# sloisel/MultiGridBarrierMPI.jl

Hardware: AMD Instinct MI355X
Metric: fem2d p-Laplace DoF/s per Newton step (higher is better)
Workload: dtype f64; 1 GPU; fem2d p-Laplace L=7 p=1 (n=57344 rows, N_L=49154 Newton unknowns), amgb main phase, tol=sqrt(eps); parallelism=single GPU

## Files before the change

### multigridbarriermpi.jl_amd/csrc/bwd_fused.cpp

```cpp
#include "bwd_fused.hpp"

#include <algorithm>

#include "chol_plan.hpp"
#include "errors.hpp"

namespace mgb {

namespace {
int round64(int v) { return (v + 63) & ~63; }
}

FusedPlan plan_bwd_fused(const CholTree& T, const FusedKnobs& kn) {
  FusedPlan P;
  const int n = T.size(), nheights = T.nheights;
  const std::vector<int>&ns = T.ns, &nf = T.nf, &first = T.first, &parent = T.parent, &height = T.height, &bofs = T.bofs;
  const std::vector<long long>&off = T.off, &loff = T.loff;
  if (kn.threads < 64 || kn.threads > 512 || (kn.threads & (kn.threads - 1))) throw ArgError("gpuchol: fused backward sweep: bad thread count");
  P.threads = kn.threads;
  P.slots.assign(T.bdry_total, -1);
  if (n == 0) return P;
  std::vector<int> hmax(nheights, 0);
  for (int t = 0; t < n; ++t) hmax[height[t]] = std::max(hmax[height[t]], nf[t]);
  int h_top = -1;
// ... 14 lines not shown
    if (parent[t] >= 0) minfirst[parent[t]] = std::min(minfirst[parent[t]], minfirst[t]);
  for (int t = n - 1; t >= 0; --t) {
    if (height[t] > h_cut) continue;
    if (parent[t] >= 0 && height[parent[t]] <= h_cut) root_of[t] = root_of[parent[t]];
    else root_of[t] = t;
  }
  for (int t = 0; t < n; ++t)
    if (root_of[t] == t) roots.push_back(t);
  std::vector<int> above(n, 0), base(n, 0);
  for (int t = n - 1; t >= 0; --t)
    if (parent[t] >= 0) above[t] = above[parent[t]] + ns[parent[t]];
  for (int t = 0; t < n; ++t) {
    const int r = root_of[t];
    if (r < 0) {
      base[t] = above[t];
      continue;
    }
    if (first[r] + ns[r] - minfirst[r] < 0 || first[t] < minfirst[r] || first[t] + ns[t] > first[r] + ns[r])
      throw InternalError("gpuchol: subtree unknowns are not contiguous");
    base[t] = above[r] + first[t] - minfirst[r];
  }
  for (int t = 0; t < n; ++t) {
    if (height[t] > h_top) continue;
    const std::vector<int>& bd = *T.bdry[t];
    int a = parent[t];
    for (size_t i = 0; i < bd.size(); ++i) {
      while (a >= 0 && !(bd[i] >= first[a] && bd[i] < first[a] + ns[a])) a = parent[a];
      if (a < 0) {
        a = parent[t];
        while (a >= 0 && !(bd[i] >= first[a] && bd[i] < first[a] + ns[a])) a = parent[a];
        if (a < 0) throw InternalError("gpuchol: boundary entry outside the ancestors");
      }
      const int ab = (root_of[a] >= 0) ? base[a] : above[a];
      P.slots[bofs[t] + i] = ab + bd[i] - first[a];
    }
  }
  auto nsl_rect = [&](int t) {
    const int h = height[t], nb = nf[t] - ns[t];
    if (nb == 0 || ns[t] == 0) return 0;
    if (hmax[h] > kn.split_nf) return 1024 / 64;
    const int nt = hmax[h] > 384 ? 1024 : 256;
    return nt / std::min(nt, round64(ns[t]));
  };
  const int W = kn.threads / 64;
  struct Rec {
    std::vector<std::vector<int>> levels;
    int first_solve = 0, sub_level = 0;
  };
  std::vector<Rec> recs(roots.size());
  std::vector<char> stored(n, 0);
  std::vector<std::vector<int>> kids(n);
  for (int t = 0; t < n; ++t)
    if (parent[t] >= 0) kids[parent[t]].push_back(t);
  size_t max_jobs = 0;
  for (size_t w = 0; w < roots.size(); ++w) {
    Rec& R = recs[w];
    const int r = roots[w];
    std::vector<int> anc;
    for (int a = parent[r]; a >= 0; a = parent[a]) anc.push_back(a);
    std::reverse(anc.begin(), anc.end());
    std::vector<int> ab;
    for (int a : anc)
      if (height[a] > h_top) ab.push_back(a);
    if (!ab.empty()) {
      R.levels.push_back(ab);
      R.first_solve = 1;
    }
    for (int a : anc)
      if (height[a] <= h_top) R.levels.push_back({a});
    R.sub_level = (int)R.levels.size();
    std::vector<int> cur{r};
    while (!cur.empty()) {
      R.levels.push_back(cur);
      std::vector<int> nxt;
      for (int t : cur) nxt.insert(nxt.end(), kids[t].begin(), kids[t].end());
      cur.swap(nxt);
    }
    size_t nj = 0;
    for (const auto& l : R.levels) nj += l.size();
    max_jobs = std::max(max_jobs, nj);
    P.max_levels = std::max(P.max_levels, (int)R.levels.size());
  }
  P.h_top = h_top;
  P.h_cut = h_cut;
  P.nwg = (int)roots.size();
  const int jo = kFusedHdr + kFusedLevelInts * P.max_levels;
  P.wstride = jo + kFusedJobInts * (int)max_jobs;
  P.wg.assign((size_t)P.nwg * P.wstride, 0);
  for (size_t w = 0; w < roots.size(); ++w) {
    const Rec& R = recs[w];
    int* rec = P.wg.data() + w * P.wstride;
    const int r = roots[w];
    int nj = 0, sl = 0;
    for (size_t l = 0; l < R.levels.size(); ++l) {
      const std::vector<int>& lv = R.levels[l];
      int* li = rec + kFusedHdr + kFusedLevelInts * l;
      const bool solve = (int)l >= R.first_solve;
      int maxp = 0, items = 0;
      li[0] = nj;
      li[1] = (int)lv.size();
      for (int t : lv) {
        int* j = rec + jo + kFusedJobInts * nj++;
        const int nsl = solve ? nsl_rect(t) : 0;
        int flags = 0;
        if (!solve) flags = 2;
        else if (root_of[t] >= 0 || !stored[t]) {
          flags = 1;
          stored[t] = 1;
        }
        j[FJ_OFF] = (int)(off[t] & 0xffffffffLL);
        j[FJ_OFF + 1] = (int)(off[t] >> 32);
        j[FJ_LOFF] = (int)(loff[t] & 0xffffffffLL);
        j[FJ_LOFF + 1] = (int)(loff[t] >> 32);
        j[FJ_FIRST] = first[t];
        j[FJ_NF] = nf[t];
        j[FJ_NS] = ns[t];
        j[FJ_SOFS] = bofs[t];
        j[FJ_BASE] = base[t];
        j[FJ_LSOFS] = sl;
        j[FJ_NSL] = nsl;
        j[FJ_NT] = hmax[height[t]] > 384 ? 1024 : 256;
        j[FJ_FLAGS] = flags;
        j[FJ_NODE] = t;
        if (solve) {
          sl += nf[t] - ns[t];
          maxp = std::max(maxp, (ns[t] + PB - 1) / PB);
          items = std::max(items, nsl * ns[t]);
        }
      }
      li[2] = maxp;
      li[3] = items;
      if (solve) {
        int G = W;
        while (G > 1 && W / G < (int)lv.size()) G >>= 1;
        P.red_cap = std::max(P.red_cap, (W / G) * items);
      }
    }
    rec[0] = (int)R.levels.size();
    rec[1] = nj;
    rec[2] = R.first_solve;
    rec[3] = above[r] + first[r] + ns[r] - minfirst[r];
    rec[4] = sl;
    rec[5] = R.sub_level;
    P.xs_cap = std::max(P.xs_cap, rec[3]);
    P.sl_cap = std::max(P.sl_cap, sl);
  }
  P.lds_bytes = (size_t)P.wstride * 4 + (size_t)(P.xs_cap + P.red_cap) * 8 + (size_t)P.sl_cap * 4;
  return P;
}

}
```

### multigridbarriermpi.jl_amd/csrc/bwd_fused.hpp

```cpp
#pragma once
#include <cstddef>
#include <vector>

namespace mgb {

struct CholTree;

struct FusedKnobs {
  int cut = 2;
  int max_wg = 256;
  int max_raise = 2;
  int top_nf = 384;
  int threads = 512;
  int split_nf = 192;
};

constexpr int kFusedHdr = 8;
constexpr int kFusedLevelInts = 4;
constexpr int kFusedJobInts = 16;
enum FusedJobField {
  FJ_OFF = 0,
  FJ_LOFF = 2,
  FJ_FIRST = 4,
  FJ_NF = 5,
  FJ_NS = 6,
  FJ_SOFS = 7,
  FJ_BASE = 8,
  FJ_LSOFS = 9,
  FJ_NSL = 10,
  FJ_NT = 11,
  FJ_FLAGS = 12,
  FJ_NODE = 13
};

struct FusedPlan {
  int h_top = -1, h_cut = -1, nwg = 0;
  int wstride = 0;
  int max_levels = 0;
  int xs_cap = 0, sl_cap = 0, red_cap = 0;
  int threads = 0;
  size_t lds_bytes = 0;
  std::vector<int> wg;
  std::vector<int> slots;
  bool enabled() const { return nwg > 0; }
};

FusedPlan plan_bwd_fused(const CholTree& T, const FusedKnobs& kn);

}
```

### multigridbarriermpi.jl_amd/csrc/chol_plan.hpp

```cpp
#pragma once
#include <algorithm>
#include <cstddef>
#include <vector>

#include "bwd_fused.hpp"
#include "chol_premap.hpp"
#include "mfchol.hpp"

namespace mgb {

constexpr int PB = 32;
constexpr int LP = PB + 1;
constexpr int TS = 64;
constexpr int TB = 256;
constexpr int RT = 1024;
constexpr int kStep2Lds = (2 * PB * PB + 3 * PB * LP + 2 * 2 * PB * (TS + 8)) * (int)sizeof(double);
constexpr int kPanel2Lds = (2 * PB * PB + 3 * PB * LP + 2 * PB * (TS + 8)) * (int)sizeof(double);
constexpr int kUpdate2Lds = (2 * 2 * PB * (TS + 8)) * (int)sizeof(double);

struct CholTree {
  int n = 0;
  double flops = 0;
  const std::vector<int>* perm = nullptr;
  std::vector<int> ns, nf, first, parent;
// ... 28 lines not shown
  long long eoff;
};

struct StartJob {
  long long off, loff;
  long long boff[2];
  int cld[2];
  int nf, ns, iofs, first;
  int node, chunk, rb;
  int a0, a1;
  long long soff[2];
};

struct StepTile {
  long long off;
  long long loff;
  int nf, ns;
  short ti, tj;
  int pad;
};

struct SingleTile {
  long long off, loff;
  long long boff[2];
  int cld[2];
  int nf, ns, iofs, a0, a1, first;
  short ti, tj;
  int pld, fofs;
  long long eoff;
  long long soff[2];
};

struct RectJob {
  int node, chunk;
};

struct CholKnobs {
  bool graph = true;
  bool prof = false;
  bool leaf = true;
  bool single = true;
  bool step2 = true;
  bool wide = true;
  bool start_pivot = true;
  int step2_tiles = 224;
  int dense_tiles = 512;
  int bwd_split_nf = 192;
  bool bwd_fused = true;
  int bwd_cut = 2;
  int bwd_fused_nf = 384;
  int bwd_fused_threads = 512;
  int premap = 1;
  int premap_tiles = 400;
};
FusedKnobs fused_knobs(const CholKnobs& kn);

enum class Kind : unsigned char {
  Leaf, Single, SingleNarrow, SingleDense, SingleDenseNarrow, Start, Step, Step2, Panel2, Update2, BwdRect, Bwd256, Bwd1024, BwdFused
};

struct Launch {
  Kind kind;
  int ofs, cnt;
  int block;
  size_t lds;
  int p, npiv;
  bool rect;
  double bytes;
  bool premap = false;
  int nproducers = 0;
};

template <class F>
int for_trailing_tiles(int nf, int k, F&& f) {
  const int Tr = (nf + 1 - k + TS - 1) / TS, Tc = std::max(1, (nf - k + TS - 1) / TS);
  int cnt = 0;
  for (int ti = 0; ti < Tr; ++ti)
    for (int tj = 0; tj <= std::min(ti, Tc - 1); ++tj, ++cnt) f(ti, tj);
  return cnt;
}
template <class F>
int for_start_jobs(int nf, F&& f) {
  int cnt = 0;
  for (int ch = 0; ch * PB < nf; ++ch)
    for (int rb = 0; rb < (nf + 1 - ch * PB + TB - 1) / TB; ++rb, ++cnt) f(ch, rb);
  return cnt;
}
inline bool has_pivot_job(bool start_pivot, int ns) { return start_pivot && ns > 0; }

struct ChainPlan {
  std::vector<GNode> nodes;
  std::vector<int> asrc, apos;
  std::vector<int> bdry;
  PremapPlan premap;
  FusedPlan fused;
  std::vector<int> lists;
  std::vector<StartJob> starts;
  std::vector<StepTile> tiles;
  std::vector<SingleTile> singles;
  std::vector<RectJob> rects;
  std::vector<Launch> chain;
  int own_bwd = 0, top_fwd = 0;
};

ChainPlan plan_chain(const CholTree& T, const CholPartition& part, int rank, const CholKnobs& kn);

// ... 2 lines not shown
```

### multigridbarriermpi.jl_amd/csrc/gpuchol.hip

```cpp
#include "gpuchol.hpp"

#include "amg.hpp"

#include <algorithm>
#include <array>
#include <cmath>
#include <cstdio>
#include <cstdlib>
#include <stdexcept>
#include <string>

namespace mgb {

namespace {

void ck(hipError_t e, const char* what) {
  if (e != hipSuccess) throw HipError(std::string("HIP error in gpuchol ") + what + ": " + hipGetErrorString(e));
}

constexpr int kProfSlots = 10;
#ifdef MGB_PROF_LAST_WG
#define MGB_PROF_WG (gridDim.x - 1)
#else
#define MGB_PROF_WG 0
// ... 1112 lines not shown
      if (k1 + r <= nf && m < kw) F[(long long)ld * (k1 + r) + k0 + m] = AT[m * TP + r];
    }
    typedef double v4f64 __attribute__((ext_vector_type(4)));
    const int lane = tid & 63, w = tid >> 6, li = lane & 15, lk = lane >> 4;
    const double* LI = AT + 16 * w + li + lk * TP;
    const double* LJ = AT + li + lk * TP;
    v4f64 acc[4];
#pragma unroll
    for (int bj = 0; bj < 4; ++bj) acc[bj] = v4f64{0.0, 0.0, 0.0, 0.0};
#pragma unroll 1
    for (int ks = 0; ks < (kw + 3) / 4; ++ks) {
      const double bv = LI[4 * ks * TP];
#pragma unroll
      for (int bj = 0; bj < 4; ++bj)
        acc[bj] = __builtin_amdgcn_mfma_f64_16x16x4f64(LJ[4 * ks * TP + 16 * bj], bv, acc[bj], 0, 0, 0);
    }
#pragma unroll
    for (int bj = 0; bj < 4; ++bj)
#pragma unroll
      for (int reg = 0; reg < 4; ++reg) {
        const int i = k1 + 16 * w + li, j = k1 + 16 * bj + lk + 4 * reg;
        if (i <= nf && j < nf && i >= j) Fs[P(i, j)] -= acc[bj][reg];
      }
    __syncthreads();
  };
  panel(0);
  if (ns > PB) panel(1);
  STAMP(2);
  const int nb = nf - ns;
  if (producer) {
    double* E = slabs + nd.eoff;
    for (int idx = tid; idx < (nb + 1) * nb; idx += TB) {
      const int a = idx % (nb + 1), q = idx / (nb + 1);
      if (a >= q) E[(long long)nd.pld * fw[q] + fw[a]] = Fs[P(ns + a, ns + q)];
    }
  } else {
    for (int idx = tid; idx < (nb + 1) * nb; idx += TB) {
      const int i = ns + idx % (nb + 1), j = ns + idx / (nb + 1);
      if (i >= j) F[(long long)ld * j + i] = Fs[P(i, j)];
    }
  }
  STAMP(7);
}

template <int NT>
__device__ inline void rect_part(const double* __restrict__ F, int ld, int ns, int nb, int j0, int jw,
                                 const double* xb, double* red, double* out , bool subtract) {
  const int tid = threadIdx.x;
  const int nsl = NT / jw, jl = tid % jw, sl = tid / jw, j = j0 + jl;
  double s = 0.0;
  if (sl < nsl && j < ns) {
    const double* col = F + (long long)ld * ns + j;
#pragma unroll 8
    for (int i = sl; i < nb; i += nsl) s = fma(col[(long long)ld * i], xb[i], s);
  }
  if (nsl > 1) {
    red[tid] = s;
    __syncthreads();
    if (sl == 0)
      for (int q = 1; q < nsl; ++q) s += red[q * jw + jl];
  }
  if (sl == 0 && j < ns) out[j] = subtract ? out[j] - s : s;
}

__global__ __launch_bounds__(RT) void backward_rect_kernel(const GNode* __restrict__ nodes, const RectJob* __restrict__ jobs,
                                                            const int* __restrict__ bdry_all,
                                                            const double* __restrict__ fronts, const double* __restrict__ y,
                                                            double* rect) {
  extern __shared__ double sh[];
  const RectJob job = jobs[blockIdx.x];
  const GNode nd = nodes[blockIdx.x];
  const int nf = nd.nf, ns = nd.ns, nb = nf - ns;
  const int* bd = bdry_all + nd.bofs;
  double* xb = sh;
  double* red = sh + nb;
  for (int i = threadIdx.x; i < nb; i += RT) xb[i] = y[bd[i]];
  __syncthreads();
  rect_part<RT>(fronts + nd.off, nf + 1, ns, nb, job.chunk * 64, 64, xb, red, rect + nd.first, false);
}

template <int NT>
__global__ __launch_bounds__(NT) void backward_kernel(const GNode* __restrict__ nodes, const int* __restrict__ list,
                                                       const int* __restrict__ bdry_all, const double* __restrict__ fronts,
                                                       const double* __restrict__ linv, const int* __restrict__ perm,
                                                       const double* __restrict__ rect, int use_rect, double* y, double* x,
                                                       long long* prof) {
  extern __shared__ double sh[];
  STAMP(0);
  const GNode nd = nodes[blockIdx.x];
  (void)list;
  const int nf = nd.nf, ns = nd.ns, nb = nf - ns, ld = nf + 1, tid = threadIdx.x;
  const double* F = fronts + nd.off;
  double* u = sh;
  double* xb = sh + ns;
  double* red = sh + nf;
  for (int i = tid; i < ns; i += NT) u[i] = F[(long long)ld * nf + i] - ((use_rect && nb > 0) ? rect[nd.first + i] : 0.0);
  STAMP(1);
  if (!use_rect && nb > 0) {
    const int* bd = bdry_all + nd.bofs;
    for (int i = tid; i < nb; i += NT) xb[i] = y[bd[i]];
    __syncthreads();
    const int jw = min(NT, (ns + 63) & ~63);
    for (int j0 = 0; j0 < ns; j0 += jw) {
      rect_part<NT>(F, ld, ns, nb, j0, jw, xb, red, u, true);
      __syncthreads();
    }
  }
// ... 90 lines not shown
}

template <int NSL>
__device__ __forceinline__ double panel_dot_lanes(const double (&f)[PB], double xq, int kw) {
  double s[NSL];
#pragma unroll
  for (int q = 0; q < NSL; ++q) s[q] = 0.0;
#pragma unroll
  for (int r = 0; r < PB; ++r) {
    const double v = fma(f[r], readlane_f64(xq, r), s[r % NSL]);
    s[r % NSL] = (r < kw) ? v : s[r % NSL];
    if (r % 8 == 7) __builtin_amdgcn_sched_barrier(0);
  }
  double t = s[0];
#pragma unroll
  for (int q = 1; q < NSL; ++q) t += s[q];
  return t;
}

__device__ inline double panel_dot_any(const double* __restrict__ Fj, long long ld, const double* up, int kw, int nsl) {
  double t = 0.0;
  for (int q = 0; q < nsl; ++q) {
    double s = 0.0;
    for (int r = q; r < kw; r += nsl) s = fma(Fj[ld * r], up[r], s);
    t = q ? t + s : s;
  }
  return t;
}

__device__ __forceinline__ double panel_update(const double (&f)[PB], bool in_f, const double* __restrict__ Fj, long long ld,
                                               const double* up, int kw, int nslp) {
  if (in_f && nslp == 1) return panel_dot<1>(f, up, kw);
  if (in_f && nslp == 2) return panel_dot<2>(f, up, kw);
  if (in_f && nslp == 4) return panel_dot<4>(f, up, kw);
  return panel_dot_any(Fj, ld, up, kw, nslp);
}

__device__ __forceinline__ void lookahead_step(double (&lc)[PB], double (&f)[PB], double& xq, const double* __restrict__ F, int ld,
                                               int ns, int nt, int q0, double* u, const double* __restrict__ lnext, int lane) {
  const int k0 = q0 - PB, qw = min(PB, ns - q0), jc = k0 + (lane & 31);
  const int jw = min(nt, (q0 + 63) & ~63), nslp = nt / jw;
  const double s = nslp == 1   ? panel_dot_lanes<1>(f, xq, qw)
                   : nslp == 2 ? panel_dot_lanes<2>(f, xq, qw)
                   : nslp == 4 ? panel_dot_lanes<4>(f, xq, qw)
                               : panel_dot_any(F + (long long)ld * q0 + jc, ld, u + q0, qw, nslp);
  if (lane < PB) u[jc] -= s;
  load_panel_rows(f, F, ld, k0, PB, k0 - PB + (lane & 31));
  xq = panel_substitute(lc, u + k0, PB, lane);
  load_pivot_block(lc, lnext, lane);
}

__device__ __forceinline__ int uni(int v) { return __builtin_amdgcn_readfirstlane(v); }

__global__ __launch_bounds__(512) void backward_fused_kernel(const int* __restrict__ wgs, int wstride, int max_levels, int xs_cap,
                                                              int red_cap, const int* __restrict__ slots,
                                                              const double* __restrict__ fronts, const double* __restrict__ linv,
                                                              const int* __restrict__ perm, double* y, double* x, long long* prof) {
  extern __shared__ double sh[];
  STAMP(0);
  int* rec = (int*)sh;
  double* xs = sh + wstride / 2;
  double* red = xs + xs_cap;
  int* sl = (int*)(red + red_cap);
  const int tid = threadIdx.x, T = blockDim.x, W = T >> 6, wave = uni(tid >> 6), lane = tid & 63;
  {
    const int* src = wgs + (size_t)blockIdx.x * wstride;
    for (int i = tid; i < wstride; i += T) rec[i] = src[i];
  }
  __syncthreads();
  const int nlevels = rec[0], njobs = rec[1], first_lv = rec[2], sub_lv = rec[5];
  const int* jobs = rec + kFusedHdr + kFusedLevelInts * max_levels;
  for (int jb = wave; jb < njobs; jb += W) {
    const int* j = jobs + kFusedJobInts * jb;
    const int nf = uni(j[FJ_NF]), ns = uni(j[FJ_NS]), flags = uni(j[FJ_FLAGS]), base = uni(j[FJ_BASE]);
    const long long off = ((long long)uni(j[FJ_OFF + 1]) << 32) | (unsigned)uni(j[FJ_OFF]);
    const double* srcv = (flags & 2) ? y + uni(j[FJ_FIRST]) : fronts + off + (long long)(nf + 1) * nf;
    for (int i0 = 0; i0 < ns; i0 += 256) {
      double v[4];
#pragma unroll
      for (int k = 0; k < 4; ++k) {
        const int i = i0 + 64 * k + lane;
        v[k] = srcv[min(i, ns - 1)];
      }
#pragma unroll
      for (int k = 0; k < 4; ++k) {
        const int i = i0 + 64 * k + lane;
        if (i < ns) xs[base + i] = v[k];
      }
    }
    if (flags & 2) continue;
    const int nb = nf - ns;
    const int* ssrc = slots + uni(j[FJ_SOFS]);
    int* sdst = sl + uni(j[FJ_LSOFS]);
    for (int i0 = 0; i0 < nb; i0 += 256) {
      int v[4];
#pragma unroll
      for (int k = 0; k < 4; ++k) {
        const int i = i0 + 64 * k + lane;
        v[k] = ssrc[min(i, nb - 1)];
      }
#pragma unroll
      for (int k = 0; k < 4; ++k) {
        const int i = i0 + 64 * k + lane;
        if (i < nb) sdst[i] = v[k];
      }
    }
  }
  __syncthreads();
  STAMP(1);
  if (first_lv == sub_lv) STAMP(2);
  for (int lv = first_lv; lv < nlevels; ++lv) {
    const int* li = rec + kFusedHdr + kFusedLevelInts * lv;
    const int lofs = li[0], cnt = li[1], maxp = li[2], items = li[3];
    int G = W;
    while (G > 1 && W / G < cnt) G >>= 1;
    const int ngrp = W / G, GT = G << 6, grp = wave / G, gtid = tid - grp * GT, gw = wave - grp * G;
    double* redg = red + grp * items;
    for (int r0 = 0; r0 < cnt; r0 += ngrp) {
      const bool act = r0 + grp < cnt;
      const int* j = jobs + kFusedJobInts * (lofs + (act ? r0 + grp : 0));
      const int nf = uni(j[FJ_NF]), ns = uni(j[FJ_NS]), nsl = uni(j[FJ_NSL]), nt = uni(j[FJ_NT]), nb = nf - ns, ld = nf + 1;
      const long long off = ((long long)uni(j[FJ_OFF + 1]) << 32) | (unsigned)uni(j[FJ_OFF]);
      const long long loff = ((long long)uni(j[FJ_LOFF + 1]) << 32) | (unsigned)uni(j[FJ_LOFF]);
      const double* F = fronts + off;
      double* u = xs + uni(j[FJ_BASE]);
      const int npanel = (ns + PB - 1) / PB;
      const bool sub = act && gw == 0 && npanel > 0;
      double lc[PB], f[PB];
      if (sub) load_pivot_block(lc, linv + loff + (long long)(npanel - 1) * 2 * PB * PB, lane);
      if (items > 0) {
        if (act && nsl > 0) {
          const int* sj = sl + uni(j[FJ_LSOFS]);
          const int nit = ns * nsl, R = (nb + nsl - 1) / nsl;
          for (int it0 = gtid; it0 < nit; it0 += 2 * GT) {
            const int it1 = it0 + GT;
            const bool has1 = it1 < nit;
            const int q0 = it0 / ns, q1 = has1 ? it1 / ns : q0;
            const double* c0 = F + (long long)ld * ns + (it0 - q0 * ns);
            const double* c1 = F + (long long)ld * ns + (has1 ? it1 - q1 * ns : it0 - q0 * ns);
            double s0 = 0.0, s1 = 0.0;
            for (int r0 = 0; r0 < R; r0 += 8) {
              double a0[8], a1[8];
#pragma unroll
              for (int k = 0; k < 8; ++k) {
                a0[k] = c0[(long long)ld * min(q0 + (r0 + k) * nsl, nb - 1)];
                a1[k] = c1[(long long)ld * min(q1 + (r0 + k) * nsl, nb - 1)];
              }
#pragma unroll
              for (int k = 0; k < 8; ++k) {
                const int i0 = q0 + (r0 + k) * nsl, i1 = q1 + (r0 + k) * nsl;
                const double v0 = fma(a0[k], xs[sj[min(i0, nb - 1)]], s0), v1 = fma(a1[k], xs[sj[min(i1, nb - 1)]], s1);
                s0 = (i0 < nb) ? v0 : s0;
                s1 = (i1 < nb) ? v1 : s1;
              }
            }
            redg[it0] = s0;
            if (has1) redg[it1] = s1;
          }
        }
        __syncthreads();
        if (act && nsl > 0)
          for (int jc = gtid; jc < ns; jc += GT) {
            double s = redg[jc];
            for (int q = 1; q < nsl; ++q) s += redg[q * ns + jc];
            u[jc] = u[jc] - s;
          }
        __syncthreads();
      }
      const bool lead = sub && G > 1 && npanel > 1;
      if (lead) {
        int k0 = (npanel - 1) * PB;
        load_panel_rows(f, F, ld, k0, ns - k0, k0 - PB + (lane & 31));
        double xq = panel_substitute(lc, u + k0, ns - k0, lane);
        load_pivot_block(lc, linv + loff + (long long)(npanel - 2) * 2 * PB * PB, lane);
        __syncthreads();
        for (int pp = npanel - 2; pp >= 0; --pp) {
          lookahead_step(lc, f, xq, F, ld, ns, nt, k0, u, linv + loff + (long long)max(pp - 1, 0) * 2 * PB * PB, lane);
          k0 -= PB;
          __syncthreads();
        }
        for (int it = npanel; it < maxp; ++it) __syncthreads();
      } else {
        const int OT = G > 1 ? GT - 64 : GT, ot = G > 1 ? gtid - 64 : gtid;
        if (act && npanel > 1) load_panel_rows(f, F, ld, (npanel - 1) * PB, ns - (npanel - 1) * PB, ot);
        for (int it = 0; it < maxp; ++it) {
          const int pp = npanel - 1 - it, k0 = pp * PB, kw = min(PB, ns - k0), q0 = k0 + PB, qw = min(PB, ns - q0);
          if (act && pp >= 0) {
            if (it > 0) {
              const int jw = min(nt, (q0 + 63) & ~63), nslp = nt / jw, hi = G > 1 ? k0 : q0;
              for (int jc = ot; jc < hi; jc += OT)
                u[jc] -= panel_update(f, jc < OT, F + (long long)ld * q0 + jc, ld, u + q0, qw, nslp);
              if (hi > PB) load_panel_rows(f, F, ld, k0, PB, ot);
            }
            if (sub) {
              panel_substitute(lc, u + k0, kw, lane);
              if (pp > 0) load_pivot_block(lc, linv + loff + (long long)(pp - 1) * 2 * PB * PB, lane);
            }
          }
          __syncthreads();
        }
      }
      if (lv >= sub_lv && act && (uni(j[FJ_FLAGS]) & 1)) {
        const int first = uni(j[FJ_FIRST]);
        for (int i = gtid; i < ns; i += GT) {
          const double v = u[i];
          y[first + i] = v;
          x[perm[first + i]] = v;
        }
      }
    }
    if (lv + 1 == sub_lv) STAMP(2);
    if (lv >= sub_lv) STAMP(min(3 + lv - sub_lv, 6));
  }
  for (int k = 3 + nlevels - sub_lv; k < 7; ++k) STAMP(k);
  const int npath = sub_lv < nlevels ? rec[kFusedHdr + kFusedLevelInts * sub_lv] : njobs;
  __syncthreads();
  for (int jb = wave; jb < npath; jb += W) {
    const int* j = jobs + kFusedJobInts * jb;
    if (!(uni(j[FJ_FLAGS]) & 1)) continue;
    const int ns = uni(j[FJ_NS]), first = uni(j[FJ_FIRST]);
    const double* u = xs + uni(j[FJ_BASE]);
    for (int i = lane; i < ns; i += 64) {
      const double v = u[i];
      y[first + i] = v;
      x[perm[first + i]] = v;
    }
  }
  STAMP(7);
}

__global__ __launch_bounds__(256) void schur_pack_kernel(const RootXchg* __restrict__ roots, const double* __restrict__ fronts,
                                                         double* __restrict__ xb) {
  const RootXchg r = roots[blockIdx.x];
  const double* F = fronts + r.off;
  for (int j = blockIdx.y; j < r.nb; j += gridDim.y) {
    double* dst = xb + r.xoff + (long long)j * (r.nb + 1) - (long long)j * (j - 1) / 2 - j;
    const double* col = F + (long long)r.ld * (r.ns + j) + r.ns;
    for (int i = j + threadIdx.x; i <= r.nb; i += blockDim.x) dst[i] = r.owned ? col[i] : 0.0;
  }
}

__global__ __launch_bounds__(256) void schur_unpack_kernel(const RootXchg* __restrict__ roots, const double* __restrict__ xb,
                                                           double* __restrict__ fronts) {
  const RootXchg r = roots[blockIdx.x];
  double* F = fronts + r.off;
  for (int j = blockIdx.y; j < r.nb; j += gridDim.y) {
    const double* src = xb + r.xoff + (long long)j * (r.nb + 1) - (long long)j * (j - 1) / 2 - j;
    double* col = F + (long long)r.ld * (r.ns + j) + r.ns;
    for (int i = j + threadIdx.x; i <= r.nb; i += blockDim.x) col[i] = src[i];
  }
}

__global__ __launch_bounds__(256) void vals_pack_kernel(int n, const int* __restrict__ idx, const double* __restrict__ vals,
                                                        double* __restrict__ xb) {
  for (int i = blockIdx.x * blockDim.x + threadIdx.x; i < n; i += gridDim.x * blockDim.x) xb[i] = vals[idx[i]];
}

__global__ __launch_bounds__(256) void vals_unpack_kernel(int n, const int* __restrict__ idx, const double* __restrict__ xb,
                                                          double* __restrict__ vals) {
  for (int i = blockIdx.x * blockDim.x + threadIdx.x; i < n; i += gridDim.x * blockDim.x) vals[idx[i]] = xb[i];
}

__global__ __launch_bounds__(256) void xsol_pack_kernel(int n, const int* __restrict__ own, const double* __restrict__ x,
                                                        const int* __restrict__ fail, double* __restrict__ xs) {
  for (long long i = (long long)blockIdx.x * blockDim.x + threadIdx.x; i <= n; i += (long long)gridDim.x * blockDim.x)
    xs[i] = (i == n) ? (*fail ? 1.0 : 0.0) : (own[i] ? x[i] : 0.0);
// ... 5 lines not shown
}

__global__ __launch_bounds__(256) void xsol_unpack_kernel(int n, const double* __restrict__ xs, double* __restrict__ x, int* fail) {
  for (long long i = (long long)blockIdx.x * blockDim.x + threadIdx.x; i <= n; i += (long long)gridDim.x * blockDim.x) {
    if (i == n) *fail = xs[n] != 0.0 ? 1 : 0;
    else x[i] = xs[i];
  }
}

}

template <class T>
T* GpuChol::upload(const std::vector<T>& v) {
  T* d = nullptr;
  const size_t bytes = std::max<size_t>(v.size(), 1) * sizeof(T);
  ck(hipMalloc((void**)&d, bytes), "hipMalloc");
  allocs_.push_back(d);
  if (!v.empty()) ck(hipMemcpy(d, v.data(), v.size() * sizeof(T), hipMemcpyHostToDevice), "H2D");
  return d;
}

GpuChol::~GpuChol() {
  for (GraphEntry& g : graphs_) (void)hipGraphExecDestroy(g.exec);
  for (void* p : allocs_) (void)hipFree(p);
}

const CholKnobs& GpuChol::knobs() {
  static const CholKnobs k = [] {
    auto on = [](const char* name) {
      const char* e = std::getenv(name);
      return !(e && e[0] == '0');
    };
    auto num = [](const char* name, int dflt) {
      const char* e = std::getenv(name);
      return e ? std::atoi(e) : dflt;
    };
    CholKnobs c;
    c.graph = on("MGB_CHOL_GRAPH");
    c.prof = std::getenv("MGB_CHOL_PROF") != nullptr;
    c.leaf = on("MGB_CHOL_LEAF");
    c.single = on("MGB_CHOL_SINGLE");
    c.step2 = on("MGB_CHOL_STEP2");
    c.wide = on("MGB_CHOL_WIDE");
    c.start_pivot = on("MGB_CHOL_START_PIVOT");
    c.step2_tiles = num("MGB_CHOL_STEP2_TILES", c.step2_tiles);
    c.dense_tiles = num("MGB_CHOL_DENSE_TILES", c.dense_tiles);
    c.bwd_split_nf = num("MGB_BWD_SPLIT_NF", c.bwd_split_nf);
    c.bwd_fused = on("MGB_CHOL_BWD_FUSED");
    c.bwd_cut = num("MGB_CHOL_BWD_CUT", c.bwd_cut);
    c.bwd_fused_nf = num("MGB_CHOL_BWD_FUSED_NF", c.bwd_fused_nf);
    c.bwd_fused_threads = num("MGB_CHOL_BWD_FUSED_THREADS", c.bwd_fused_threads);
    c.premap = num("MGB_CHOL_PREMAP", c.premap);
    c.premap_tiles = num("MGB_CHOL_PREMAP_TILES", c.premap_tiles);
    return c;
  }();
  return k;
}

void GpuChol::schedule_info(int cap, int* nlaunch, int* kind, int* workgroups) const {
  if (nlaunch) *nlaunch = (int)chain_.size();
  const int m = std::min(std::max(cap, 0), (int)chain_.size());
  for (int i = 0; i < m; ++i) {
    if (kind) kind[i] = (int)chain_[i].kind;
    if (workgroups) workgroups[i] = chain_[i].cnt;
  }
}

void GpuChol::premap_info(int cap, int* consumer, int* producers) const {
  const int m = std::min(std::max(cap, 0), (int)chain_.size());
  for (int i = 0; i < m; ++i) {
    if (consumer) consumer[i] = chain_[i].premap ? 1 : 0;
    if (producers) producers[i] = chain_[i].nproducers;
  }
}

void GpuChol::unknown_columns(const MfChol& sym, int* node, int* col) {
  const CholTree T = sym.view();
  for (int t = 0; t < T.size(); ++t)
    for (int k = 0; k < T.ns[t]; ++k) {
      const int i = (*T.perm)[T.first[t] + k];
      if (node) node[i] = t;
      if (col) col[i] = k;
    }
}

void GpuChol::build(const MfChol& sym, Ctx* ctx) {
  ctx_ = ctx;
  part_ = (ctx && ctx->world > 1) ? sym.partition(ctx->world) : CholPartition();
  const int my_rank = ctx ? ctx->rank : 0;
  const CholTree T = sym.view();
  ChainPlan P = plan_chain(T, part_, my_rank, knobs());
  const std::vector<GNode>& nodes = P.nodes;
  const std::vector<int>& perm = *T.perm;
  const int nnodes = T.size();
  n_ = T.n;
  flops_ = T.flops;
  total_front_ = T.front_doubles;
  chain_ = std::move(P.chain);
  own_bwd_ = P.own_bwd;
  top_fwd_ = P.top_fwd;
  premap_ = std::move(P.premap);
  fused_ = std::move(P.fused);
  d_nodes_ = upload(nodes);
  d_perm_ = upload(perm);
  d_bdry_ = upload(P.bdry);
  d_pinv_ = upload(premap_.pinv);
// ... 145 lines not shown
}
}

void GpuChol::run(hipStream_t st, int begin, int end, const double* d_vals, const double* d_b, double* d_x, KernelTimer* tm) {
  for (int i = begin; i < end; ++i) {
    const Launch& L = chain_[i];
    if (L.cnt == 0) continue;
    long long* prof = d_prof_ ? d_prof_ + (size_t)kProfSlots * i : nullptr;
    const dim3 grid(L.cnt), block(L.block);
    const bool narrow = L.kind == Kind::SingleNarrow || L.kind == Kind::SingleDenseNarrow;
    const bool dense = L.kind == Kind::SingleDense || L.kind == Kind::SingleDenseNarrow;
    if (tm) tm->begin(st, timer_class(L.kind), L.bytes);
    switch (L.kind) {
      case Kind::Leaf:
        hipLaunchKernelGGL(front_leaf_kernel, grid, block, L.lds, st, d_hnodes_ + L.ofs, d_lists_ + L.ofs, d_asm_src_, d_asm_pos_,
                           d_vals, d_perm_, d_b, d_fronts_, d_linv_, d_fail_, prof, d_slabs_, d_fwd_);
        break;
      case Kind::Single:
      case Kind::SingleNarrow:
      case Kind::SingleDense:
      case Kind::SingleDenseNarrow:
        hipLaunchKernelGGL(L.premap ? (dense ? (narrow ? front_single_dense_kernel<true, true> : front_single_dense_kernel<false, true>)
                                             : (narrow ? front_single_kernel<true, true> : front_single_kernel<false, true>))
                                    : (dense ? (narrow ? front_single_dense_kernel<true, false> : front_single_dense_kernel<false, false>)
                                             : (narrow ? front_single_kernel<true, false> : front_single_kernel<false, false>)),
                           grid, block, L.lds, st, d_singles_ + L.ofs, d_pinv_, d_asm_src_, d_asm_pos_, d_vals, d_perm_, d_b, d_fronts_,
                           d_fronts_, d_linv_, d_fail_, prof, d_slabs_, d_slabs_, d_fwd_);
        break;
      case Kind::Start:
        hipLaunchKernelGGL(L.premap ? front_start_kernel<true> : front_start_kernel<false>, grid, block, L.lds, st, d_nodes_,
                           d_start_ + L.ofs, d_pinv_, d_asm_src_, d_asm_pos_, d_vals, d_perm_, d_b, d_fronts_, d_fronts_, d_linv_,
                           d_fail_, prof, knobs().start_pivot ? 1 : 0, d_slabs_);
        break;
      case Kind::Step:
      case Kind::Step2:
      case Kind::Panel2:
      case Kind::Update2:
        hipLaunchKernelGGL(L.kind == Kind::Step ? front_step_kernel : L.kind == Kind::Step2 ? front_step2_kernel
                           : L.kind == Kind::Panel2 ? front_panel2_kernel : front_update2_kernel,
                           grid, block, L.lds, st, d_tiles_ + L.ofs, L.p, L.npiv, d_fronts_, d_linv_, d_linv_, d_fail_, prof);
        break;
      case Kind::BwdRect:
        hipLaunchKernelGGL(backward_rect_kernel, grid, block, L.lds, st, d_rnodes_ + L.ofs, d_rectjobs_ + L.ofs, d_bdry_, d_fronts_,
                           d_y_, d_rect_);
        break;
      case Kind::Bwd256:
      case Kind::Bwd1024:
        hipLaunchKernelGGL(L.kind == Kind::Bwd1024 ? backward_kernel<1024> : backward_kernel<256>, grid, block, L.lds, st,
                           d_hnodes_ + L.ofs, d_lists_ + L.ofs, d_bdry_, d_fronts_, d_linv_, d_perm_, d_rect_, L.rect ? 1 : 0, d_y_,
                           d_x, prof);
        break;
      case Kind::BwdFused:
        hipLaunchKernelGGL(backward_fused_kernel, grid, block, L.lds, st, d_fused_wg_, fused_.wstride, fused_.max_levels,
                           fused_.xs_cap, fused_.red_cap, d_fused_slots_, d_fronts_, d_linv_, d_perm_, d_y_, d_x, prof);
        break;
    }
    if (tm) tm->end(st);
  }
}

void GpuChol::enqueue_chain(hipStream_t st, const double* d_vals, const double* d_b, double* d_x) {
  if (part_.split()) throw InternalError("gpuchol: a split factorisation cannot be captured");
  if (n_ == 0) return;
  run(st, 0, top_fwd_, d_vals, d_b, d_x, nullptr);
  ck(hipGetLastError(), "chain launches");
}

void GpuChol::factor_solve_split(hipStream_t st, double* d_vals, const double* d_b, double* d_x, KernelTimer* tm, bool values_summed,
                                 bool x_local) {
  const bool ride = vals_local_ && !values_summed;
  const int ntop = ride ? ntop_vals_ : 0;
  run(st, 0, own_bwd_, d_vals, d_b, d_x, tm);
  const dim3 xg(nroots_, std::max(1, std::min(64, max_root_nb_)));
  hipLaunchKernelGGL(schur_pack_kernel, xg, dim3(256), 0, st, d_roots_, d_fronts_, d_xchg_);
  const int vgrid = std::max(1, std::min(1024, (ntop_vals_ + 255) / 256));
  if (ride)
    hipLaunchKernelGGL(vals_pack_kernel, dim3(vgrid), dim3(256), 0, st, ntop_vals_, d_top_idx_, d_vals, d_xchg_ + xchg_doubles_);
  ck(hipGetLastError(), "schur pack");
  ctx_->allreduce_sum(d_xchg_, xchg_doubles_ + ntop);
  hipLaunchKernelGGL(schur_unpack_kernel, xg, dim3(256), 0, st, d_roots_, d_xchg_, d_fronts_);
  if (ride)
    hipLaunchKernelGGL(vals_unpack_kernel, dim3(vgrid), dim3(256), 0, st, ntop_vals_, d_top_idx_, d_xchg_ + xchg_doubles_, d_vals);
  run(st, top_fwd_, (int)chain_.size(), d_vals, d_b, d_x, tm);
  run(st, own_bwd_, top_fwd_, d_vals, d_b, d_x, tm);
  const int grid = std::min(2048, (n_ + 256) / 256);
  if (x_local) {
    hipLaunchKernelGGL(x_local_kernel, dim3(grid), dim3(256), 0, st, n_, d_kind_orig_, d_x);
    ck(hipGetLastError(), "x_local");
    return;
  }
  hipLaunchKernelGGL(xsol_pack_kernel, dim3(grid), dim3(256), 0, st, n_, d_own_orig_, d_x, d_fail_, d_xsol_);
  ck(hipGetLastError(), "xsol pack");
  ctx_->allreduce_sum(d_xsol_, (long long)n_ + 1);
  hipLaunchKernelGGL(xsol_unpack_kernel, dim3(grid), dim3(256), 0, st, n_, d_xsol_, d_x, d_fail_);
  ck(hipGetLastError(), "factor_solve_split launches");
}

void GpuChol::enqueue(hipStream_t st, const double* d_vals, const double* d_b, double* d_x, KernelTimer* tm) {
  run(st, 0, top_fwd_, d_vals, d_b, d_x, tm);
  ck(hipGetLastError(), "factor_solve launches");
  if (d_prof_) print_stamps(st);
}

void GpuChol::reset_stamps() {
  std::vector<long long> init((size_t)kProfSlots * chain_.size(), 0LL);
  for (size_t q = 0; q < chain_.size(); ++q) init[kProfSlots * q + 8] = -1LL;
  ck(hipMemcpy(d_prof_, init.data(), init.size() * sizeof(long long), hipMemcpyHostToDevice), "prof reset");
// ... 62 lines not shown
```

Baseline: 92.72 million DoF/s per Newton step.

## Overlap next level's rectangular update with current panel solve in fused backward sweep

In the fused backward triangular-solve kernel, wave 0 now runs the serial panel substitution on the ancestor path alone. The other waves meanwhile load and accumulate the next child node's off-diagonal contributions, using unknowns as each panel finishes. The host plan stores per-panel boundary ranges so those waves know which entries are ready, and the rectangular dot-product loops run in reverse row order so partial sums match that schedule. The aim is to hide the next level's memory-bound update behind the latency-bound substitution chain. The cost is register pressure from the look-ahead state, more complex control flow, and a changed summation order.

```diff
diff --git a/multigridbarriermpi.jl_amd/csrc/bwd_fused.cpp b/multigridbarriermpi.jl_amd/csrc/bwd_fused.cpp
--- a/multigridbarriermpi.jl_amd/csrc/bwd_fused.cpp
+++ b/multigridbarriermpi.jl_amd/csrc/bwd_fused.cpp
@@ -90,7 +90,25 @@
   std::vector<std::vector<int>> kids(n);
   for (int t = 0; t < n; ++t)
     if (parent[t] >= 0) kids[parent[t]].push_back(t);
-  size_t max_jobs = 0;
+  auto panel_ranges = [&](int d, int f, std::vector<int>& r) {
+    const std::vector<int>& bd = *T.bdry[d];
+    const int lo = first[f], hi = first[f] + ns[f], np = (ns[f] + PB - 1) / PB;
+    size_t npar = 0;
+    while (npar < bd.size() && bd[npar] >= lo && bd[npar] < hi && (npar == 0 || bd[npar] > bd[npar - 1])) ++npar;
+    for (size_t i = npar; i < bd.size(); ++i)
+      if (bd[i] >= lo && bd[i] < hi) return false;
+    r.assign(np + 1, (int)npar);
+    for (int p = 0, i = 0; p < np; ++p) {
+      while (i < (int)npar && bd[i] - lo < p * PB) ++i;
+      r[p] = i;
+    }
+    return nf[d] > ns[d] && ns[d] > 0 && np > 0;
+  };
+  auto ahead_level = [](const Rec& R, size_t l) {
+    return (int)l > R.first_solve && (int)l < R.sub_level && R.levels[l - 1].size() == 1;
+  };
+  size_t max_jobs = 0, max_ranges = 0;
+  std::vector<int> rg;
   for (size_t w = 0; w < roots.size(); ++w) {
     Rec& R = recs[w];
     const int r = roots[w];
@@ -117,19 +135,24 @@
     size_t nj = 0;
     for (const auto& l : R.levels) nj += l.size();
     max_jobs = std::max(max_jobs, nj);
+    size_t nr = 0;
+    for (size_t l = 0; l < R.levels.size(); ++l)
+      if (ahead_level(R, l) && panel_ranges(R.levels[l][0], R.levels[l - 1][0], rg)) nr += rg.size();
+    max_ranges = std::max(max_ranges, nr);
     P.max_levels = std::max(P.max_levels, (int)R.levels.size());
   }
   P.h_top = h_top;
   P.h_cut = h_cut;
   P.nwg = (int)roots.size();
   const int jo = kFusedHdr + kFusedLevelInts * P.max_levels;
-  P.wstride = jo + kFusedJobInts * (int)max_jobs;
+  const int ro = jo + kFusedJobInts * (int)max_jobs;
+  P.wstride = (ro + (int)max_ranges + 1) & ~1;
   P.wg.assign((size_t)P.nwg * P.wstride, 0);
   for (size_t w = 0; w < roots.size(); ++w) {
     const Rec& R = recs[w];
     int* rec = P.wg.data() + w * P.wstride;
     const int r = roots[w];
-    int nj = 0, sl = 0;
+    int nj = 0, sl = 0, rpos = ro;
     for (size_t l = 0; l < R.levels.size(); ++l) {
       const std::vector<int>& lv = R.levels[l];
       int* li = rec + kFusedHdr + kFusedLevelInts * l;
@@ -160,6 +183,14 @@
         j[FJ_NT] = hmax[height[t]] > 384 ? 1024 : 256;
         j[FJ_FLAGS] = flags;
         j[FJ_NODE] = t;
+        j[FJ_AOFS] = 0;
+        j[FJ_APAR] = 0;
+        if (ahead_level(R, l) && panel_ranges(t, R.levels[l - 1][0], rg)) {
+          j[FJ_AOFS] = rpos;
+          j[FJ_APAR] = rg.back();
+          std::copy(rg.begin(), rg.end(), rec + rpos);
+          rpos += (int)rg.size();
+        }
         if (solve) {
           sl += nf[t] - ns[t];
           maxp = std::max(maxp, (ns[t] + PB - 1) / PB);
diff --git a/multigridbarriermpi.jl_amd/csrc/bwd_fused.hpp b/multigridbarriermpi.jl_amd/csrc/bwd_fused.hpp
--- a/multigridbarriermpi.jl_amd/csrc/bwd_fused.hpp
+++ b/multigridbarriermpi.jl_amd/csrc/bwd_fused.hpp
@@ -30,7 +30,9 @@
   FJ_NSL = 10,
   FJ_NT = 11,
   FJ_FLAGS = 12,
-  FJ_NODE = 13
+  FJ_NODE = 13,
+  FJ_AOFS = 14,
+  FJ_APAR = 15
 };
 
 struct FusedPlan {
diff --git a/multigridbarriermpi.jl_amd/csrc/chol_plan.hpp b/multigridbarriermpi.jl_amd/csrc/chol_plan.hpp
--- a/multigridbarriermpi.jl_amd/csrc/chol_plan.hpp
+++ b/multigridbarriermpi.jl_amd/csrc/chol_plan.hpp
@@ -104,6 +104,7 @@
   int bwd_fused_threads = 512;
   int premap = 1;
   int premap_tiles = 400;
+  bool bwd_ahead = true;
 };
 FusedKnobs fused_knobs(const CholKnobs& kn);
 
diff --git a/multigridbarriermpi.jl_amd/csrc/gpuchol.hip b/multigridbarriermpi.jl_amd/csrc/gpuchol.hip
--- a/multigridbarriermpi.jl_amd/csrc/gpuchol.hip
+++ b/multigridbarriermpi.jl_amd/csrc/gpuchol.hip
@@ -1188,7 +1188,7 @@
   if (sl < nsl && j < ns) {
     const double* col = F + (long long)ld * ns + j;
 #pragma unroll 8
-    for (int i = sl; i < nb; i += nsl) s = fma(col[(long long)ld * i], xb[i], s);
+    for (int i = sl + (nb - 1 - sl) / nsl * nsl; i >= sl && i < nb; i -= nsl) s = fma(col[(long long)ld * i], xb[i], s);
   }
   if (nsl > 1) {
     red[tid] = s;
@@ -1385,10 +1385,68 @@
 
 __device__ __forceinline__ int uni(int v) { return __builtin_amdgcn_readfirstlane(v); }
 
+constexpr int kAheadItems = 5;
+constexpr int kAheadRows = 4;
+
+struct AheadPart {
+  double s[kAheadItems];
+  double a[kAheadItems][kAheadRows];
+  int n[kAheadItems];
+  int jc[kAheadItems];
+};
+
+__device__ __forceinline__ void ahead_begin(AheadPart& A, int ot, int OT, int ns, int nb, int nsl) {
+  const int m = (nb - 1) / nsl, rem = nb - 1 - m * nsl;
+#pragma unroll
+  for (int k = 0; k < kAheadItems; ++k) {
+    const int it = ot + k * OT;
+    const bool has = it < ns * nsl;
+    const int q = has ? it / ns : 0;
+    A.jc[k] = has ? it - q * ns : 0;
+    A.n[k] = has ? q + (q <= rem ? m : m - 1) * nsl : -1;
+    A.s[k] = 0.0;
+  }
+}
+
+__device__ __forceinline__ void ahead_load(AheadPart& A, const double* __restrict__ C, int ld, int nb, int nsl) {
+#pragma unroll
+  for (int k = 0; k < kAheadItems; ++k)
+#pragma unroll
+    for (int r = 0; r < kAheadRows; ++r) A.a[k][r] = C[(long long)ld * min(max(A.n[k] - r * nsl, 0), nb - 1) + A.jc[k]];
+}
+
+__device__ __forceinline__ void ahead_add(AheadPart& A, const double* xs, const int* sj, int lo, int nsl) {
+#pragma unroll
+  for (int k = 0; k < kAheadItems; ++k) {
+    int n = A.n[k];
+#pragma unroll
+    for (int r = 0; r < kAheadRows; ++r) {
+      const int i = A.n[k] - r * nsl;
+      const double v = fma(A.a[k][r], xs[sj[max(i, 0)]], A.s[k]);
+      A.s[k] = (i >= lo) ? v : A.s[k];
+      n = (i >= lo) ? i - nsl : n;
+    }
+    A.n[k] = n;
+  }
+}
+
+template <bool MORE>
+__device__ __forceinline__ void ahead_window(AheadPart& A, const double* __restrict__ C, int ld, int nb, int nsl, const double* xs,
+                                             const int* sj, int lo, int hi) {
+  if (hi <= lo) return;
+  ahead_add(A, xs, sj, lo, nsl);
+  for (int done = kAheadRows * nsl; done < hi - lo; done += kAheadRows * nsl) {
+    ahead_load(A, C, ld, nb, nsl);
+    ahead_add(A, xs, sj, lo, nsl);
+  }
+  if (MORE) ahead_load(A, C, ld, nb, nsl);
+}
+
 __global__ __launch_bounds__(512) void backward_fused_kernel(const int* __restrict__ wgs, int wstride, int max_levels, int xs_cap,
                                                               int red_cap, const int* __restrict__ slots,
                                                               const double* __restrict__ fronts, const double* __restrict__ linv,
-                                                              const int* __restrict__ perm, double* y, double* x, long long* prof) {
+                                                              const int* __restrict__ perm, double* y, double* x, long long* prof,
+                                                              int ahead) {
   extern __shared__ double sh[];
   STAMP(0);
   int* rec = (int*)sh;
@@ -1442,7 +1500,12 @@
   __syncthreads();
   STAMP(1);
   if (first_lv == sub_lv) STAMP(2);
-  for (int lv = first_lv; lv < nlevels; ++lv) {
+  AheadPart A = {};
+  bool held = false;
+  int a_pos = 0;
+  constexpr int kAll = 0, kLead = 1, kOthers = 2;
+  auto level = [&](const int lv, auto role_) {
+    constexpr int ROLE = decltype(role_)::value;
     const int* li = rec + kFusedHdr + kFusedLevelInts * lv;
     const int lofs = li[0], cnt = li[1], maxp = li[2], items = li[3];
     int G = W;
@@ -1460,9 +1523,19 @@
       const int npanel = (ns + PB - 1) / PB;
       const bool sub = act && gw == 0 && npanel > 0;
       double lc[PB], f[PB];
-      if (sub) load_pivot_block(lc, linv + loff + (long long)(npanel - 1) * 2 * PB * PB, lane);
+      if constexpr (ROLE != kOthers) {
+        if (sub) load_pivot_block(lc, linv + loff + (long long)(npanel - 1) * 2 * PB * PB, lane);
+      }
+      const int OT = G > 1 ? GT - 64 : GT, ot = G > 1 ? gtid - 64 : gtid;
       if (items > 0) {
-        if (act && nsl > 0) {
+        if (act && nsl > 0 && held) {
+          if constexpr (ROLE == kOthers) {
+            ahead_window<false>(A, F + (long long)ld * ns, ld, nb, nsl, xs, sl + uni(j[FJ_LSOFS]), 0, a_pos);
+#pragma unroll
+            for (int k = 0; k < kAheadItems; ++k)
+              if (ot + k * OT < ns * nsl) redg[ot + k * OT] = A.s[k];
+          }
+        } else if (act && nsl > 0) {
           const int* sj = sl + uni(j[FJ_LSOFS]);
           const int nit = ns * nsl, R = (nb + nsl - 1) / nsl;
           for (int it0 = gtid; it0 < nit; it0 += 2 * GT) {
@@ -1476,15 +1549,15 @@
               double a0[8], a1[8];
 #pragma unroll
               for (int k = 0; k < 8; ++k) {
-                a0[k] = c0[(long long)ld * min(q0 + (r0 + k) * nsl, nb - 1)];
-                a1[k] = c1[(long long)ld * min(q1 + (r0 + k) * nsl, nb - 1)];
+                a0[k] = c0[(long long)ld * min(max(q0 + (R - 1 - r0 - k) * nsl, 0), nb - 1)];
+                a1[k] = c1[(long long)ld * min(max(q1 + (R - 1 - r0 - k) * nsl, 0), nb - 1)];
               }
 #pragma unroll
               for (int k = 0; k < 8; ++k) {
-                const int i0 = q0 + (r0 + k) * nsl, i1 = q1 + (r0 + k) * nsl;
-                const double v0 = fma(a0[k], xs[sj[min(i0, nb - 1)]], s0), v1 = fma(a1[k], xs[sj[min(i1, nb - 1)]], s1);
-                s0 = (i0 < nb) ? v0 : s0;
-                s1 = (i1 < nb) ? v1 : s1;
+                const int i0 = q0 + (R - 1 - r0 - k) * nsl, i1 = q1 + (R - 1 - r0 - k) * nsl;
+                const double v0 = fma(a0[k], xs[sj[min(max(i0, 0), nb - 1)]], s0), v1 = fma(a1[k], xs[sj[min(max(i1, 0), nb - 1)]], s1);
+                s0 = (r0 + k < R && i0 < nb) ? v0 : s0;
+                s1 = (r0 + k < R && i1 < nb) ? v1 : s1;
               }
             }
             redg[it0] = s0;
@@ -1501,7 +1574,65 @@
         __syncthreads();
       }
       const bool lead = sub && G > 1 && npanel > 1;
-      if (lead) {
+      bool ahead_d = false;
+      const int* jd = j + kFusedJobInts;
+      const int *rg = rec, *sjd = sl;
+      const double* Cd = F;
+      int d_ld = 0, d_nb = 0, d_nsl = 0, d_par = 0;
+      if (ROLE != kAll && npanel > 0 && lv + 1 < sub_lv) {
+        const int aofs = uni(jd[FJ_AOFS]), d_ns = uni(jd[FJ_NS]);
+        d_nsl = uni(jd[FJ_NSL]);
+        d_nb = uni(jd[FJ_NF]) - d_ns;
+        ahead_d = aofs > 0 && d_nsl > 0 && d_ns * d_nsl <= kAheadItems * OT;
+        if (ahead_d) {
+          rg = rec + aofs;
+          sjd = sl + uni(jd[FJ_LSOFS]);
+          d_par = uni(jd[FJ_APAR]);
+          d_ld = d_nb + d_ns + 1;
+          const long long d_off = ((long long)uni(jd[FJ_OFF + 1]) << 32) | (unsigned)uni(jd[FJ_OFF]);
+          Cd = fronts + d_off + (long long)d_ld * d_ns;
+          if constexpr (ROLE == kOthers) {
+            ahead_begin(A, ot, OT, d_ns, d_nb, d_nsl);
+            ahead_load(A, Cd, d_ld, d_nb, d_nsl);
+          }
+          a_pos = d_nb;
+        }
+      }
+      auto panels = [&](auto role) {
+        constexpr bool SUBST = decltype(role)::value;
+        if (act && npanel > 1) load_panel_rows(f, F, ld, (npanel - 1) * PB, ns - (npanel - 1) * PB, ot);
+        for (int it = 0; it < maxp; ++it) {
+          const int pp = npanel - 1 - it, k0 = pp * PB, kw = min(PB, ns - k0), q0 = k0 + PB, qw = min(PB, ns - q0);
+          if (act && pp >= 0) {
+            if (it > 0) {
+              const int jw = min(nt, (q0 + 63) & ~63), nslp = nt / jw, hi = G > 1 ? k0 : q0;
+              for (int jc = ot; jc < hi; jc += OT)
+                u[jc] -= panel_update(f, jc < OT, F + (long long)ld * q0 + jc, ld, u + q0, qw, nslp);
+              if (hi > PB) load_panel_rows(f, F, ld, k0, PB, ot);
+            }
+            if constexpr (SUBST) {
+              if (sub) {
+                panel_substitute(lc, u + k0, kw, lane);
+                if (pp > 0) load_pivot_block(lc, linv + loff + (long long)(pp - 1) * 2 * PB * PB, lane);
+              }
+            }
+          }
+          if constexpr (!SUBST) {
+            if (ahead_d) {
+              const int lo = max(it == 0 ? d_par : uni(rg[npanel - it]), a_pos - kAheadRows * d_nsl);
+              if (lo < a_pos) {
+                ahead_add(A, xs, sjd, lo, d_nsl);
+                ahead_load(A, Cd, d_ld, d_nb, d_nsl);
+              }
+              a_pos = lo;
+            }
+          }
+          __syncthreads();
+        }
+      };
+      if constexpr (ROLE == kOthers) {
+        panels(std::false_type{});
+      } else if (lead) {
         int k0 = (npanel - 1) * PB;
         load_panel_rows(f, F, ld, k0, ns - k0, k0 - PB + (lane & 31));
         double xq = panel_substitute(lc, u + k0, ns - k0, lane);
@@ -1514,24 +1645,7 @@
         }
         for (int it = npanel; it < maxp; ++it) __syncthreads();
       } else {
-        const int OT = G > 1 ? GT - 64 : GT, ot = G > 1 ? gtid - 64 : gtid;
-        if (act && npanel > 1) load_panel_rows(f, F, ld, (npanel - 1) * PB, ns - (npanel - 1) * PB, ot);
-        for (int it = 0; it < maxp; ++it) {
-          const int pp = npanel - 1 - it, k0 = pp * PB, kw = min(PB, ns - k0), q0 = k0 + PB, qw = min(PB, ns - q0);
-          if (act && pp >= 0) {
-            if (it > 0) {
-              const int jw = min(nt, (q0 + 63) & ~63), nslp = nt / jw, hi = G > 1 ? k0 : q0;
-              for (int jc = ot; jc < hi; jc += OT)
-                u[jc] -= panel_update(f, jc < OT, F + (long long)ld * q0 + jc, ld, u + q0, qw, nslp);
-              if (hi > PB) load_panel_rows(f, F, ld, k0, PB, ot);
-            }
-            if (sub) {
-              panel_substitute(lc, u + k0, kw, lane);
-              if (pp > 0) load_pivot_block(lc, linv + loff + (long long)(pp - 1) * 2 * PB * PB, lane);
-            }
-          }
-          __syncthreads();
-        }
+        panels(std::true_type{});
       }
       if (lv >= sub_lv && act && (uni(j[FJ_FLAGS]) & 1)) {
         const int first = uni(j[FJ_FIRST]);
@@ -1541,10 +1655,19 @@
           x[perm[first + i]] = v;
         }
       }
+      held = ahead_d;
     }
     if (lv + 1 == sub_lv) STAMP(2);
     if (lv >= sub_lv) STAMP(min(3 + lv - sub_lv, 6));
-  }
+  };
+  int lv = first_lv;
+  if (ahead && W > 1) {
+    if (wave == 0)
+      for (; lv < sub_lv; ++lv) level(lv, std::integral_constant<int, kLead>{});
+    else
+      for (; lv < sub_lv; ++lv) level(lv, std::integral_constant<int, kOthers>{});
+  }
+  for (; lv < nlevels; ++lv) level(lv, std::integral_constant<int, kAll>{});
   for (int k = 3 + nlevels - sub_lv; k < 7; ++k) STAMP(k);
   const int npath = sub_lv < nlevels ? rec[kFusedHdr + kFusedLevelInts * sub_lv] : njobs;
   __syncthreads();
@@ -1656,6 +1779,7 @@
     c.bwd_fused_threads = num("MGB_CHOL_BWD_FUSED_THREADS", c.bwd_fused_threads);
     c.premap = num("MGB_CHOL_PREMAP", c.premap);
     c.premap_tiles = num("MGB_CHOL_PREMAP_TILES", c.premap_tiles);
+    c.bwd_ahead = on("MGB_CHOL_BWD_AHEAD");
     return c;
   }();
   return k;
@@ -1907,7 +2031,8 @@
         break;
       case Kind::BwdFused:
         hipLaunchKernelGGL(backward_fused_kernel, grid, block, L.lds, st, d_fused_wg_, fused_.wstride, fused_.max_levels,
-                           fused_.xs_cap, fused_.red_cap, d_fused_slots_, d_fronts_, d_linv_, d_perm_, d_y_, d_x, prof);
+                           fused_.xs_cap, fused_.red_cap, d_fused_slots_, d_fronts_, d_linv_, d_perm_, d_y_, d_x, prof,
+                           knobs().bwd_ahead ? 1 : 0);
         break;
     }
     if (tm) tm->end(st);
```

Result: slower. 89.89 million DoF/s per Newton step (-3.1%).
